# Person-Recognition-for-Pose-Estimation/Person-Recognition-for-Pose-Estimation

Measured on AMD Instinct MI355X. Metric: frames/sec whole-node, 640×640 bs=256, 1/2/4/8 MI355X; OKS Δ vs CPU ref, higher is better.
Workload: dtype f32 storage/accumulate; split-operand MFMA: trunk 2x fp16 planes (3 terms), YOLO net 3x bf16 (6 terms), YOLO / ViT adapters and ViT 2x bf16 (3 terms), AdaFace adapter 3x3s + IR-50 1x fp16 plane with per-frame power-of-2 scaling (1 term); 1 GPU; full multi-task model (trunk + face-YOLO + AdaFace + ViTPose + NMS + soft-argmax), 640x640; global_batch=256, per_gpu_batch=256, parallelism=dp1 (frame sharding, RCCL all-gather of detections), world_size_observed=1, precision_policy=auto

## Files before the change

person-recognition-for-pose-estimation_amd/csrc/conv_halo.hip:

```cpp
#include "conv.h"

namespace prpe_k {
namespace {

constexpr int HBK = 32;


template <int NTN, int K>
__device__ __forceinline__ void slab_gemm(const float* ct, int cs, const uint16_t* w, int ws, int ps, int fr, int fg,
                                          f32x4 (&zc)[NTN]) {
#pragma unroll
  for (int jn = 0; jn < NTN; ++jn) zc[jn] = f32x4{0.f, 0.f, 0.f, 0.f};
#pragma unroll
  for (int kk = 0; kk < K / 32; ++kk) {
    const float* ap = ct + fr * cs + kk * 32 + fg * 8;
    bf16x4 p0[2], p1[2];
    split_planes<2>(*reinterpret_cast<const f4*>(ap), p0);
    split_planes<2>(*reinterpret_cast<const f4*>(ap + 4), p1);
    bf16x8 za[2];
#pragma unroll
    for (int q = 0; q < 2; ++q)
      za[q] = bf16x8{p0[q][0], p0[q][1], p0[q][2], p0[q][3], p1[q][0], p1[q][1], p1[q][2], p1[q][3]};
#pragma unroll
    for (int jn = 0; jn < NTN; ++jn) {
      const uint16_t* bp = w + (jn * 16 + fr) * ws + kk * 32 + fg * 8;
      const bf16x8 b0 = *reinterpret_cast<const bf16x8*>(bp);
      const bf16x8 b1 = *reinterpret_cast<const bf16x8*>(bp + ps);
      zc[jn] = mfma16(za[1], b0, zc[jn]);
      zc[jn] = mfma16(za[0], b1, zc[jn]);
      zc[jn] = mfma16(za[0], b0, zc[jn]);
    }
  }
}

template <int R, int C>
__device__ __forceinline__ void stage_planes(const float* w, int rows, int cols, int ld, uint16_t* dst, int ws,
                                             int tid, int nthr) {
  for (int e = tid; e < R * C / 4; e += nthr) {
    const int r = e / (C / 4), c = (e - r * (C / 4)) * 4;
    f4 v = {0.f, 0.f, 0.f, 0.f};
    if (r < rows && c < cols) v = *reinterpret_cast<const f4*>(w + r * ld + c);
    bf16x4 pl[2];
    split_planes<2>(v, pl);
    *reinterpret_cast<bf16x4*>(dst + r * ws + c) = pl[0];
    *reinterpret_cast<bf16x4*>(dst + R * ws + r * ws + c) = pl[1];
  }
}

template <int NW, int TR, int TC, int TN, bool F16, bool APL, int TAPS = 0, int WN = 1, bool ONE = false>
__global__ __launch_bounds__(NW * 64) __attribute__((amdgpu_waves_per_eu(2))) void conv_halo_kernel(ConvK p, int tiles_w, int tiles_h) {
  static_assert(TC % 16 == 0 && (TR * TC / 16) % (NW / WN) == 0 && TN % WN == 0, "tile");
  static_assert(!(F16 && APL), "planes input is precision 0");
  static_assert(!ONE || (F16 && TAPS == 0), "single fp16 plane: precision 4, no epilogue GEMM");
  static_assert(WN == 1 || WN == 2, "waves along N");
  using frag_t = typename std::conditional<F16, f16x8, bf16x8>::type;
  constexpr int TM = TR * TC / 16 / (NW / WN);
  constexpr int TNW = TN / WN;
  constexpr int BN = TN * 16, NP = ONE ? 1 : 2;
  constexpr int HW_ = TC + 2, HP = (TR + 2) * HW_;
  constexpr int HQ = (HP + 7) / 8;
  constexpr int HALO = HQ * 8 * 128;
  constexpr int B_STAGE = NP * BN * 64;
  constexpr int NB_TOT = NP * BN / 16;
  constexpr int IB = NB_TOT / NW;
  static_assert(NB_TOT % NW == 0, "B pieces per wave");
  constexpr int CS = BN / WN + 4;
  constexpr int EPI = NW * 16 * CS * 4;
  constexpr int H16 = ONE ? HQ * 8 * 64 : 0;
  constexpr int MAIN = 2 * HALO + 2 * B_STAGE + H16;
  constexpr int W2R = TAPS == 2 ? 64 : 32;
  constexpr int W2B = TAPS ? 2 * W2R * (BN + 8) * 2 + (TAPS == 2 ? 2 * 32 * 72 * 2 : 0) : 0;
  constexpr int LDS_BYTES = MAIN > EPI + W2B ? MAIN : EPI + W2B;
  __shared__ __attribute__((aligned(1024))) unsigned char lds[LDS_BYTES];
  unsigned char* const halo0 = lds;
  unsigned char* const ring = lds + 2 * HALO;
  unsigned char* const h16 = lds + 2 * HALO + 2 * B_STAGE;

  const int tid = threadIdx.x, lane = tid & 63, wave = __builtin_amdgcn_readfirstlane(tid >> 6);
  const int wm = wave / WN, wn = wave % WN;
  const int fr = lane & 15, fg = lane >> 4;
  int L = xcd_remap(blockIdx.x, p.nwg);
  const int tile_n = L % p.tiles_n;
  L /= p.tiles_n;
  const int tw = L % tiles_w;
  L /= tiles_w;
  const int th = L % tiles_h;
  const int n = L / tiles_h;
  const int n0 = tile_n * BN;
  const int oh0 = th * TR, ow0 = tw * TC;

  constexpr unsigned OOB = 0x80000000u;
  const float* xn = p.x + (int64_t)n * p.xsn;
  const int frame_bytes = (int)(((int64_t)(p.Hi - 1) * p.xsh + (int64_t)(p.Wi - 1) * p.xsw + p.Ci) * 4);
  const __amdgpu_buffer_rsrc_t xr = buf_rsrc(xn, frame_bytes);
  constexpr int KQ = (HQ + NW - 1) / NW;
  unsigned hvo[KQ];
#pragma unroll
  for (int k = 0; k < KQ; ++k) {
    const int q = wave + k * NW;
    const int px = q * 8 + (lane >> 3);
    const int hr = px / HW_, hc = px - hr * HW_;
    const int ih = oh0 - 1 + hr, iw = ow0 - 1 + hc;
    const int sl = (lane & 7) ^ swz_halo(hc);
    const bool ok = q < HQ && px < HP && (unsigned)ih < (unsigned)p.Hi && (unsigned)iw < (unsigned)p.Wi;
    hvo[k] = ok ? (unsigned)(((int64_t)ih * p.xsh + (int64_t)iw * p.xsw + sl * 4) * 4) : OOB;
  }
  auto issue_halo = [&](int k, int c, int buf) {
    bl_lds16_nt(xr, halo0 + buf * HALO + (wave + k * NW) * 1024, hvo[k], c * HBK * 4);
  };

  const int wbytes = p.k_pad * 2 * (p.tiles_n * BN);
  const __amdgpu_buffer_rsrc_t wr0 = buf_rsrc(F16 ? p.wh16 : p.whi, wbytes);
  const __amdgpu_buffer_rsrc_t wr1 = buf_rsrc(F16 ? p.wl16 : p.wlo, wbytes);
  unsigned bvo[IB];
  int bdst[IB];
  bool bpl[IB];
#pragma unroll
  for (int i = 0; i < IB; ++i) {
    const int j = wave * IB + i;
    const int q = j / (BN / 16), rb = j % (BN / 16);
    const int nrow = rb * 16 + (lane >> 2);
    const int ch = (lane & 3) ^ swzF(nrow);
    bvo[i] = (unsigned)(((n0 + nrow) * p.k_pad + ch * 8) * 2);
    bdst[i] = (q * BN + rb * 16) * 64;
    bpl[i] = q != 0;
  }
  auto issue_b = [&](int kt, int stage) {
    unsigned char* sb = ring + stage * B_STAGE;
#pragma unroll
    for (int i = 0; i < IB; ++i)
      bl_lds16(bpl[i] ? wr1 : wr0, sb + bdst[i], bvo[i], kt * HBK * 2);
  };

  const bool pro = ONE && p.in_scale != nullptr;
  float sa = 1.f, inv = 1.f;
  if constexpr (F16) {
    float am = p.x_amax[n];
    if (pro) {
      float pS, pB;
      prologue_bounds(p.in_scale, p.in_bias, p.Ci, pS, pB);
      am = fmaf(am, pS, pB);
    }
    const int e = f16_scale_exp(am);
    sa = ldexpf(1.f, 15 - e);
    inv = ldexpf(1.f, e - 15);
  }

  int aoff[TM][9];
#pragma unroll
  for (int i = 0; i < TM; ++i) {
    const int rb = wm * TM + i;
    const int hb0 = (rb / (TC / 16)) * HW_ + (rb % (TC / 16)) * 16 + fr;
#pragma unroll
    for (int t = 0; t < 9; ++t) {
      const int px = hb0 + (t / 3) * HW_ + t % 3;
      const int sw = swz_halo(px % HW_);
      aoff[i][t] = ONE ? px * 64 + ((fg ^ ((px >> 2) & 3)) << 4) : px * 128 + (((2 * fg) ^ sw) << 4);
    }
  }

  f32x4 acc[TM][TNW];
#pragma unroll
  for (int i = 0; i < TM; ++i)
#pragma unroll
    for (int j = 0; j < TNW; ++j) acc[i][j] = f32x4{0.f, 0.f, 0.f, 0.f};

  const int nc = p.Ci / HBK;
  const int nk = nc * 9;
#pragma unroll
  for (int k = 0; k < KQ; ++k)
    if (wave + k * NW < HQ) issue_halo(k, 0, 0);
  issue_b(0, 0);

#pragma unroll 1
  for (int c = 0; c < nc; ++c) {
    const unsigned char* hb = halo0 + (c & 1) * HALO;
    const int kt0 = c * 9;
#pragma unroll
    for (int t = 0; t < 9; ++t) {
      const int kt = kt0 + t;
      wait_barrier<0>();
      if (kt + 1 < nk) issue_b(kt + 1, (kt + 1) & 1);
      if (c + 1 < nc) {
#pragma unroll
        for (int k = t; k < KQ; k += 9)
          if (wave + k * NW < HQ) issue_halo(k, c + 1, (c + 1) & 1);
      }
      if constexpr (ONE) {
        if (t == 0) {
          f4 ps4[2], pb4[2];
          if (pro) {
            const int ch = c * HBK + (tid & 3) * 8;
#pragma unroll
            for (int h = 0; h < 2; ++h) {
              ps4[h] = *reinterpret_cast<const f4*>(p.in_scale + ch + 4 * h);
              pb4[h] = *reinterpret_cast<const f4*>(p.in_bias + ch + 4 * h);
            }
          }
          for (int e = tid; e < HP * 4; e += NW * 64) {
            const int q = e >> 2, g = e & 3;
            const int hr = q / HW_, hc = q - hr * HW_;
            const int sw = swz_halo(hc);
            f4 v0 = *reinterpret_cast<const f4*>(hb + q * 128 + (((2 * g) ^ sw) << 4));
            f4 v1 = *reinterpret_cast<const f4*>(hb + q * 128 + (((2 * g + 1) ^ sw) << 4));
            if (pro) {
              const bool in = (unsigned)(oh0 - 1 + hr) < (unsigned)p.Hi && (unsigned)(ow0 - 1 + hc) < (unsigned)p.Wi;
              v0 = in ? affine4(v0, ps4[0], pb4[0]) : f4{0.f, 0.f, 0.f, 0.f};
              v1 = in ? affine4(v1, ps4[1], pb4[1]) : f4{0.f, 0.f, 0.f, 0.f};
            }
            *reinterpret_cast<f16x8*>(h16 + q * 64 + ((g ^ ((q >> 2) & 3)) << 4)) = cvt_f16_one(v0, v1, sa);
          }
          __builtin_amdgcn_sched_barrier(0);
          asm volatile("s_waitcnt lgkmcnt(0)\n\ts_barrier" ::: "memory");
          __builtin_amdgcn_sched_barrier(0);
        }
      }
      frag_t af[NP][TM];
#pragma unroll
      for (int i = 0; i < TM; ++i) {
        if constexpr (ONE) {
          af[0][i] = *reinterpret_cast<const f16x8*>(h16 + aoff[i][t]);
          continue;
        }
        const f4 v0 = *reinterpret_cast<const f4*>(hb + aoff[i][t]);
        const f4 v1 = *reinterpret_cast<const f4*>(hb + (aoff[i][t] ^ 16));
        if constexpr (APL) {
          af[0][i] = __builtin_bit_cast(bf16x8, v0);
          af[1][i] = __builtin_bit_cast(bf16x8, v1);
        } else if constexpr (ONE) {
          af[0][i] = cvt_f16_one(v0, v1, sa);
        } else if constexpr (F16) {
          unsigned long long p0[2], p1[2];
          split_planes_f16(v0, sa, p0);
          split_planes_f16(v1, sa, p1);
#pragma unroll
          for (int q = 0; q < 2; ++q) {
            typedef unsigned long long u64x2 __attribute__((ext_vector_type(2)));
            af[q][i] = __builtin_bit_cast(f16x8, u64x2{p0[q], p1[q]});
          }
        } else {
          bf16x4 p0[NP], p1[NP];
          split_planes<NP>(v0, p0);
          split_planes<NP>(v1, p1);
#pragma unroll
          for (int q = 0; q < NP; ++q)
            af[q][i] = bf16x8{p0[q][0], p0[q][1], p0[q][2], p0[q][3], p1[q][0], p1[q][1], p1[q][2], p1[q][3]};
        }
      }
      const unsigned char* sb = ring + (kt & 1) * B_STAGE;
#pragma unroll
      for (int j = 0; j < TNW; ++j) {
        const int nrow = (wn * TNW + j) * 16 + fr;
        const unsigned char* bp = sb + nrow * 64 + ((fg ^ swzF(nrow)) << 4);
        frag_t bfr[NP];
#pragma unroll
        for (int q = 0; q < NP; ++q) bfr[q] = *reinterpret_cast<const frag_t*>(bp + q * BN * 64);
#pragma unroll
        for (int i = 0; i < TM; ++i)
#pragma unroll
          for (int s = NP - 1; s >= 0; --s)
#pragma unroll
            for (int qa = s; qa >= 0; --qa) acc[i][j] = mfma16(af[qa][i], bfr[s - qa], acc[i][j]);
      }
    }
  }
  wait_barrier<0>();

  float* ct = reinterpret_cast<float*>(lds) + wave * 16 * CS;
  constexpr int CPR = BN / WN / 4;
  constexpr int RPP = 64 / CPR;
  constexpr int EB = 16 / RPP;
  const int cc = lane % CPR, rr0 = lane / CPR;
  const int col = n0 + wn * (BN / WN) + cc * 4;
  const bool cval = col < p.Co;
  f4 sc4 = {1.f, 1.f, 1.f, 1.f}, bi4 = {0.f, 0.f, 0.f, 0.f}, sl4 = {0.f, 0.f, 0.f, 0.f};
  if (cval) {
    if (p.scale) sc4 = *reinterpret_cast<const f4*>(p.scale + col);
    if (p.bias) bi4 = *reinterpret_cast<const f4*>(p.bias + col);
    if (p.slope) sl4 = *reinterpret_cast<const f4*>(p.slope + col);
  }
  float ym = 0.f;
  constexpr int W2S = BN + 8, W3S = 72;
  uint16_t* const w2s = reinterpret_cast<uint16_t*>(lds + EPI);
  uint16_t* const w3s = w2s + 2 * W2R * W2S;
  if constexpr (TAPS != 0) {
    stage_planes<W2R, BN>(p.w2, TAPS == 2 ? p.nmid : p.n2, p.Co, p.Co, w2s, W2S, tid, NW * 64);
    if constexpr (TAPS == 2) stage_planes<32, 64>(p.w3, p.n2, p.nmid, p.nmid, w3s, W3S, tid, NW * 64);
    __syncthreads();
  }
  f32x4 s2 = {0.f, 0.f, 0.f, 0.f}, b2 = {0.f, 0.f, 0.f, 0.f};
  if constexpr (TAPS == 2) {
#pragma unroll
    for (int jn = 0; jn < 4; ++jn) {
      const int c = jn * 16 + fr;
      if (c < p.nmid) {
        s2[jn] = p.s2 ? p.s2[c] : 1.f;
        b2[jn] = p.b2 ? p.b2[c] : 0.f;
      }
    }
  }
#pragma unroll
  for (int i = 0; i < TM; ++i) {
    const int rb = wm * TM + i;
    const int oh = oh0 + rb / (TC / 16), owb = ow0 + (rb % (TC / 16)) * 16;
#pragma unroll
    for (int r = 0; r < 4; ++r)
#pragma unroll
      for (int j = 0; j < TNW; ++j) ct[(fg * 4 + r) * CS + j * 16 + fr] = acc[i][j][r];
    int64_t yo[EB];
    f4 res[EB];
    bool ok[EB];
#pragma unroll
    for (int e = 0; e < EB; ++e) {
      const int ow = owb + rr0 + RPP * e;
      ok[e] = cval && oh < p.Ho && ow < p.Wo;
      res[e] = f4{0.f, 0.f, 0.f, 0.f};
      yo[e] = 0;
      if (ok[e]) {
        yo[e] = (int64_t)n * p.ysn + (int64_t)oh * p.ysh + (int64_t)ow * p.ysw + col;
        if (p.res_mode != PRPE_RES_NONE)
          res[e] = *reinterpret_cast<const f4*>(p.r + (int64_t)n * p.rsn + (int64_t)oh * p.rsh + (int64_t)ow * p.rsw + col);
      }
    }
#pragma unroll(ONE ? 2 : EB)
    for (int e = 0; e < EB; ++e) {
      f4 v = *reinterpret_cast<const f4*>(ct + (rr0 + RPP * e) * CS + cc * 4);
      if (!ok[e]) continue;
      if constexpr (F16) v = v * inv;
      v = v * sc4 + bi4;
      if (p.res_mode == PRPE_RES_PRE_ACT) v += res[e];
      v = apply_act4(v, p.act, sl4);
      if (p.res_mode == PRPE_RES_POST_ACT) v += res[e];
      if constexpr (TAPS != 0) {
        *reinterpret_cast<f4*>(ct + (rr0 + RPP * e) * CS + cc * 4) = v;
        continue;
      }
      if (p.y_planes) {
        bf16x4 pl[2];
        split_planes<2>(v, pl);
        uint16_t* y16 = reinterpret_cast<uint16_t*>(p.y) + 2 * (yo[e] - col) + (col >> 3) * 16 + (col & 7);
        *reinterpret_cast<bf16x4*>(y16) = pl[0];
        *reinterpret_cast<bf16x4*>(y16 + 8) = pl[1];
      } else {
        *reinterpret_cast<f4*>(p.y + yo[e]) = v;
      }
      if (p.y_amax) ym = fmaxf(ym, amax4(v));
    }
    if constexpr (TAPS != 0) {
      __builtin_amdgcn_wave_barrier();
      constexpr int KH = BN / WN;
      const uint16_t* w2w = w2s + wn * KH;
      auto hand_over = [&](auto& part, auto nt) {
        constexpr int NT_ = decltype(nt)::value;
        if (wn == 1) {
#pragma unroll
          for (int jn = 0; jn < NT_; ++jn)
#pragma unroll
            for (int r = 0; r < 4; ++r) ct[(fg * 4 + r) * CS + jn * 16 + fr] = part[jn][r];
        }
        __syncthreads();
        if (wn == 0) {
          const float* pc = ct + 16 * CS;
#pragma unroll
          for (int jn = 0; jn < NT_; ++jn)
#pragma unroll
            for (int r = 0; r < 4; ++r) part[jn][r] += pc[(fg * 4 + r) * CS + jn * 16 + fr];
        }
      };
      f32x4 zc[2];
      if constexpr (TAPS == 1) {
        slab_gemm<2, KH>(ct, CS, w2w, W2S, W2R * W2S, fr, fg, zc);
        if constexpr (WN == 2) hand_over(zc, std::integral_constant<int, 2>{});
      } else {
        f32x4 zm[4];
        slab_gemm<4, KH>(ct, CS, w2w, W2S, W2R * W2S, fr, fg, zm);
        if constexpr (WN == 2) hand_over(zm, std::integral_constant<int, 4>{});
        __builtin_amdgcn_wave_barrier();
        if (wn == 0) {
#pragma unroll
          for (int jn = 0; jn < 4; ++jn) {
            const f32x4 t = apply_act4(zm[jn] * s2[jn] + b2[jn], p.act2, f32x4{0.f, 0.f, 0.f, 0.f});
#pragma unroll
            for (int r = 0; r < 4; ++r) ct[(fg * 4 + r) * CS + jn * 16 + fr] = t[r];
          }
          __builtin_amdgcn_wave_barrier();
          slab_gemm<2, 64>(ct, CS, w3s, W3S, 32 * W3S, fr, fg, zc);
        }
      }
      if (wn == 0) {
#pragma unroll
        for (int r = 0; r < 4; ++r) {
          const int ow = owb + fg * 4 + r;
          if (oh < p.Ho && ow < p.Wo) {
            float* zo = p.y2 + (int64_t)n * p.y2sn + (int64_t)oh * p.y2sh + (int64_t)ow * p.y2sw;
#pragma unroll
            for (int jn = 0; jn < 2; ++jn)
              if (jn * 16 + fr < p.n2) zo[jn * 16 + fr] = zc[jn][r];
          }
        }
      }
      if constexpr (WN == 2) __syncthreads();
      __builtin_amdgcn_wave_barrier();
    }
  }
  if (p.y_amax) amax_commit(p.y_amax + n, ym);
}

template <int NW, int TR, int TC, int TN, bool F16, bool APL, int TAPS = 0, int WN = 1, bool ONE = false>
int launch_halo(const ConvK& kp0, hipStream_t st) {
  ConvK kp = kp0;
  if (kp.w2 && kp.Co > TN * 16) return PRPE_EINVAL;
  const int tiles_w = (kp.Wo + TC - 1) / TC, tiles_h = (kp.Ho + TR - 1) / TR;
  kp.tiles_n = (kp.Co + TN * 16 - 1) / (TN * 16);
  const int64_t nwg = (int64_t)(kp.M / kp.HoWo) * tiles_h * tiles_w * kp.tiles_n;
  if (nwg <= 0 || nwg >= (1LL << 31)) return PRPE_EINVAL;
  kp.nwg = (int)nwg;
  hipLaunchKernelGGL((conv_halo_kernel<NW, TR, TC, TN, F16, APL, TAPS, WN, ONE>), dim3(kp.nwg), dim3(NW * 64), 0, st,
                     kp, tiles_w, tiles_h);
  return launch_status();
}

template <int NW, int TR, int TC, int TN, int WN = 1>
int launch_halo_kind(const ConvK& kp, int prec, hipStream_t st) {
  if (prec == 3) return launch_halo<NW, TR, TC, TN, true, false, 0, WN>(kp, st);
  if constexpr ((TN * 16 / 16) % NW == 0)
    if (prec == 4) return launch_halo<NW, TR, TC, TN, true, false, 0, WN, true>(kp, st);
  if (prec == 4) return PRPE_EINVAL;
  return kp.x_planes ? launch_halo<NW, TR, TC, TN, false, true, 0, WN>(kp, st)
                     : launch_halo<NW, TR, TC, TN, false, false, 0, WN>(kp, st);
}

template <int TAPS, int NW>
int launch_halo_taps(const ConvK& kp, int prec, hipStream_t st) {
  constexpr int TR = NW == 4 ? 8 : 16;
  if (prec == 4) return PRPE_EINVAL;
  if (prec == 3) return launch_halo<NW, TR, 16, 8, true, false, TAPS>(kp, st);
  return kp.x_planes ? launch_halo<NW, TR, 16, 8, false, true, TAPS>(kp, st)
                     : launch_halo<NW, TR, 16, 8, false, false, TAPS>(kp, st);
}

}

bool conv_halo_eligible(const ConvK& kp, int prec, int km, int tile) {
  const bool p3 = prec == 3 && kp.wh16 && kp.wl16 && kp.x_amax && !kp.x_planes;
  const bool p4 = prec == 4 && kp.wh16 && kp.x_amax && !kp.x_planes && (!kp.in_scale || kp.in_bias) && tile != 35 &&
                  !kp.w2;
  const int64_t frame_bytes = ((int64_t)(kp.Hi - 1) * kp.xsh + (int64_t)(kp.Wi - 1) * kp.xsw + kp.Ci) * 4;
  const int64_t w_bytes = (int64_t)kp.k_pad * 2 * (((kp.Co + 127) / 128) * 128);
  return km == 2 && kp.KH == 3 && kp.KW == 3 && kp.stride == 1 && kp.pad == 1 && kp.Ci % HBK == 0 &&
         kp.vec_out && (prec == 0 || p3 || p4) && (!kp.in_scale || p4) && !kp.x2 && kp.k_pad == kp.K && kp.zero &&
         kp.Hi == kp.Ho && kp.Wi == kp.Wo && kp.xsh >= 0 && kp.xsw >= 0 && frame_bytes < (1LL << 31) &&
         w_bytes < (1LL << 31);
}

bool conv_halo_auto(const ConvK& kp, int prec) {
  if (prec == 4 && kp.Ho >= 14 && kp.Wo >= 14) return true;
  if (prec == 0 && !kp.x_planes) return false;
  const int tc = 16, tr = 8;
  const int64_t covered = (int64_t)((kp.Ho + tr - 1) / tr) * tr * ((kp.Wo + tc - 1) / tc) * tc;
  return covered * 20 <= (int64_t)kp.Ho * kp.Wo * 21;
}

int conv_halo_launch(const ConvK& kp, int prec, int tile, hipStream_t st) {
  if (kp.w2) {
    if (tile == 32) return kp.w3 ? launch_halo_taps<2, 8>(kp, prec, st) : launch_halo_taps<1, 8>(kp, prec, st);
    if (tile != 30 && tile != 31) return PRPE_EINVAL;
    return kp.w3 ? launch_halo_taps<2, 4>(kp, prec, st) : launch_halo_taps<1, 4>(kp, prec, st);
  }
  if (tile == 30) tile = kp.Co <= 64 ? 34 : (prec == 4 ? 36 : 31);
  switch (tile) {
    case 31: return launch_halo_kind<4, 8, 16, 8>(kp, prec, st);
    case 32: return launch_halo_kind<8, 16, 16, 8>(kp, prec, st);
    case 33: return launch_halo_kind<8, 8, 32, 8>(kp, prec, st);
    case 34: return launch_halo_kind<4, 8, 16, 4>(kp, prec, st);
    case 35: return launch_halo_kind<8, 16, 16, 4>(kp, prec, st);
    case 36: return launch_halo_kind<4, 8, 16, 8, 2>(kp, prec, st);
    case 37: return launch_halo_kind<8, 16, 16, 8, 2>(kp, prec, st);
    default: return PRPE_EINVAL;
  }
}

}
```

Measured before the change: 1679 frames/sec.

## Unroll halo conv channel loop by parity and simplify halo/weight load addressing

After: 1679 frames/sec, median of 6. Within noise of the previous version (+0.0%).

```diff
diff --git a/person-recognition-for-pose-estimation_amd/csrc/conv_halo.hip b/person-recognition-for-pose-estimation_amd/csrc/conv_halo.hip
--- a/person-recognition-for-pose-estimation_amd/csrc/conv_halo.hip
+++ b/person-recognition-for-pose-estimation_amd/csrc/conv_halo.hip
@@ -94,42 +94,41 @@
   const int frame_bytes = (int)(((int64_t)(p.Hi - 1) * p.xsh + (int64_t)(p.Wi - 1) * p.xsw + p.Ci) * 4);
   const __amdgpu_buffer_rsrc_t xr = buf_rsrc(xn, frame_bytes);
   constexpr int KQ = (HQ + NW - 1) / NW;
+  static_assert(KQ >= 2, "halo pieces per wave");
+  const int hq_last = wave + (KQ - 1) * NW < HQ ? wave + (KQ - 1) * NW : wave + (KQ - 2) * NW;
   unsigned hvo[KQ];
 #pragma unroll
   for (int k = 0; k < KQ; ++k) {
-    const int q = wave + k * NW;
+    const int q = k == KQ - 1 ? hq_last : wave + k * NW;
     const int px = q * 8 + (lane >> 3);
     const int hr = px / HW_, hc = px - hr * HW_;
     const int ih = oh0 - 1 + hr, iw = ow0 - 1 + hc;
     const int sl = (lane & 7) ^ swz_halo(hc);
-    const bool ok = q < HQ && px < HP && (unsigned)ih < (unsigned)p.Hi && (unsigned)iw < (unsigned)p.Wi;
+    const bool ok = px < HP && (unsigned)ih < (unsigned)p.Hi && (unsigned)iw < (unsigned)p.Wi;
     hvo[k] = ok ? (unsigned)(((int64_t)ih * p.xsh + (int64_t)iw * p.xsw + sl * 4) * 4) : OOB;
   }
   auto issue_halo = [&](int k, int c, int buf) {
-    bl_lds16_nt(xr, halo0 + buf * HALO + (wave + k * NW) * 1024, hvo[k], c * HBK * 4);
+    const int q = k == KQ - 1 ? hq_last : wave + k * NW;
+    bl_lds16_nt(xr, halo0 + buf * HALO + q * 1024, hvo[k], c * HBK * 4);
   };
 
+  static_assert(TN % IB == 0, "a wave's B pieces in one plane");
   const int wbytes = p.k_pad * 2 * (p.tiles_n * BN);
-  const __amdgpu_buffer_rsrc_t wr0 = buf_rsrc(F16 ? p.wh16 : p.whi, wbytes);
-  const __amdgpu_buffer_rsrc_t wr1 = buf_rsrc(F16 ? p.wl16 : p.wlo, wbytes);
+  const int bq = wave * IB / TN, rb0 = wave * IB % TN;
+  const void* wpl = F16 ? (const void*)p.wh16 : (const void*)p.whi;
+  if (NP == 2 && bq != 0) wpl = F16 ? (const void*)p.wl16 : (const void*)p.wlo;
+  const __amdgpu_buffer_rsrc_t wr = buf_rsrc(wpl, wbytes);
   unsigned bvo[IB];
-  int bdst[IB];
-  bool bpl[IB];
 #pragma unroll
   for (int i = 0; i < IB; ++i) {
-    const int j = wave * IB + i;
-    const int q = j / (BN / 16), rb = j % (BN / 16);
-    const int nrow = rb * 16 + (lane >> 2);
+    const int nrow = (rb0 + i) * 16 + (lane >> 2);
     const int ch = (lane & 3) ^ swzF(nrow);
     bvo[i] = (unsigned)(((n0 + nrow) * p.k_pad + ch * 8) * 2);
-    bdst[i] = (q * BN + rb * 16) * 64;
-    bpl[i] = q != 0;
-  }
+  }
+  unsigned char* const bdst = ring + (bq * BN + rb0 * 16) * 64;
   auto issue_b = [&](int kt, int stage) {
-    unsigned char* sb = ring + stage * B_STAGE;
-#pragma unroll
-    for (int i = 0; i < IB; ++i)
-      bl_lds16(bpl[i] ? wr1 : wr0, sb + bdst[i], bvo[i], kt * HBK * 2);
+#pragma unroll
+    for (int i = 0; i < IB; ++i) bl_lds16(wr, bdst + stage * B_STAGE + i * 1024, bvo[i], kt * HBK * 2);
   };
 
   const bool pro = ONE && p.in_scale != nullptr;
@@ -166,26 +165,27 @@
     for (int j = 0; j < TNW; ++j) acc[i][j] = f32x4{0.f, 0.f, 0.f, 0.f};
 
   const int nc = p.Ci / HBK;
-  const int nk = nc * 9;
-#pragma unroll
-  for (int k = 0; k < KQ; ++k)
-    if (wave + k * NW < HQ) issue_halo(k, 0, 0);
+#pragma unroll
+  for (int k = 0; k < KQ; ++k) issue_halo(k, 0, 0);
   issue_b(0, 0);
 
-#pragma unroll 1
-  for (int c = 0; c < nc; ++c) {
-    const unsigned char* hb = halo0 + (c & 1) * HALO;
-    const int kt0 = c * 9;
+  auto chunk = [&](const int c, auto par_c, auto tail_c) {
+    constexpr int PAR = decltype(par_c)::value;
+    constexpr bool TAIL = decltype(tail_c)::value;
+    const unsigned char* hb = halo0 + PAR * HALO;
 #pragma unroll
     for (int t = 0; t < 9; ++t) {
-      const int kt = kt0 + t;
+      const int kt = c * 9 + t;
+      const int st = (PAR + t) & 1;
+      auto issue_next = [&] {
+        if (!TAIL || t < 8) issue_b(kt + 1, st ^ 1);
+        if (!TAIL) {
+#pragma unroll
+          for (int k = t; k < KQ; k += 9) issue_halo(k, c + 1, PAR ^ 1);
+        }
+      };
       wait_barrier<0>();
-      if (kt + 1 < nk) issue_b(kt + 1, (kt + 1) & 1);
-      if (c + 1 < nc) {
-#pragma unroll
-        for (int k = t; k < KQ; k += 9)
-          if (wave + k * NW < HQ) issue_halo(k, c + 1, (c + 1) & 1);
-      }
+      issue_next();
       if constexpr (ONE) {
         if (t == 0) {
           f4 ps4[2], pb4[2];
@@ -210,25 +210,36 @@
             }
             *reinterpret_cast<f16x8*>(h16 + q * 64 + ((g ^ ((q >> 2) & 3)) << 4)) = cvt_f16_one(v0, v1, sa);
           }
-          __builtin_amdgcn_sched_barrier(0);
-          asm volatile("s_waitcnt lgkmcnt(0)\n\ts_barrier" ::: "memory");
-          __builtin_amdgcn_sched_barrier(0);
+          lds_barrier();
         }
       }
       frag_t af[NP][TM];
+      f4 av[ONE ? 1 : TM][2];
 #pragma unroll
       for (int i = 0; i < TM; ++i) {
         if constexpr (ONE) {
           af[0][i] = *reinterpret_cast<const f16x8*>(h16 + aoff[i][t]);
-          continue;
-        }
-        const f4 v0 = *reinterpret_cast<const f4*>(hb + aoff[i][t]);
-        const f4 v1 = *reinterpret_cast<const f4*>(hb + (aoff[i][t] ^ 16));
+        } else {
+          av[i][0] = *reinterpret_cast<const f4*>(hb + aoff[i][t]);
+          av[i][1] = *reinterpret_cast<const f4*>(hb + (aoff[i][t] ^ 16));
+        }
+      }
+      const unsigned char* sb = ring + st * B_STAGE;
+      auto read_b = [&](int j, frag_t (&bfr)[NP]) {
+        const int nrow = (wn * TNW + j) * 16 + fr;
+        const unsigned char* bp = sb + nrow * 64 + ((fg ^ swzF(nrow)) << 4);
+#pragma unroll
+        for (int q = 0; q < NP; ++q) bfr[q] = *reinterpret_cast<const frag_t*>(bp + q * BN * 64);
+      };
+      frag_t bf0[NP];
+      read_b(0, bf0);
+#pragma unroll
+      for (int i = 0; i < TM; ++i) {
+        if constexpr (ONE) continue;
+        const f4 v0 = av[ONE ? 0 : i][0], v1 = av[ONE ? 0 : i][1];
         if constexpr (APL) {
           af[0][i] = __builtin_bit_cast(bf16x8, v0);
           af[1][i] = __builtin_bit_cast(bf16x8, v1);
-        } else if constexpr (ONE) {
-          af[0][i] = cvt_f16_one(v0, v1, sa);
         } else if constexpr (F16) {
           unsigned long long p0[2], p1[2];
           split_planes_f16(v0, sa, p0);
@@ -247,14 +258,15 @@
             af[q][i] = bf16x8{p0[q][0], p0[q][1], p0[q][2], p0[q][3], p1[q][0], p1[q][1], p1[q][2], p1[q][3]};
         }
       }
-      const unsigned char* sb = ring + (kt & 1) * B_STAGE;
 #pragma unroll
       for (int j = 0; j < TNW; ++j) {
-        const int nrow = (wn * TNW + j) * 16 + fr;
-        const unsigned char* bp = sb + nrow * 64 + ((fg ^ swzF(nrow)) << 4);
         frag_t bfr[NP];
-#pragma unroll
-        for (int q = 0; q < NP; ++q) bfr[q] = *reinterpret_cast<const frag_t*>(bp + q * BN * 64);
+        if (j == 0) {
+#pragma unroll
+          for (int q = 0; q < NP; ++q) bfr[q] = bf0[q];
+        } else {
+          read_b(j, bfr);
+        }
 #pragma unroll
         for (int i = 0; i < TM; ++i)
 #pragma unroll
@@ -263,6 +275,20 @@
             for (int qa = s; qa >= 0; --qa) acc[i][j] = mfma16(af[qa][i], bfr[s - qa], acc[i][j]);
       }
     }
+  };
+  using even_t = std::integral_constant<int, 0>;
+  using odd_t = std::integral_constant<int, 1>;
+  int c = 0;
+#pragma unroll 1
+  for (; c + 2 < nc; c += 2) {
+    chunk(c, even_t{}, std::false_type{});
+    chunk(c + 1, odd_t{}, std::false_type{});
+  }
+  if (c + 2 == nc) {
+    chunk(c, even_t{}, std::false_type{});
+    chunk(c + 1, odd_t{}, std::true_type{});
+  } else {
+    chunk(c, even_t{}, std::true_type{});
   }
   wait_barrier<0>();
 
```
